# shayneobrien/generative-models

Hardware: AMD Instinct MI355X
Metric: images/sec (28x28 MNIST) per D+G step, NSGAN bs=256 (higher is better)
Workload: dtype f32; 1 GPU; NSGAN MNIST bs=256 fp32 per GPU (BASELINE.json configs[1]); 784-400-20 MLPs, N=50000 synthetic Bernoulli images, parity-mode RNG protocol, Adam 2e-4, D_steps=1; global_batch=256, parallelism=dp1, ranks_seen=1, gradient_exchange=none (1 rank), timing=one 2064-step timed region, cold_start_inclusive=False

## Files before the change

generative_models_amd/csrc/gm_gemm.hip:

```cpp
#include "gm_common.h"
#include "gm_head.h"
#include "gm_gather.h"
#include "gm_dvae.h"
#include "gm_ldsdma.h"

#include <cstdlib>
#include <type_traits>

typedef float f32x16 __attribute__((ext_vector_type(16)));

#ifdef GM_STAMPS
namespace gm_stamps {
constexpr int WAVES = 16, IDS = 40, HDR = 8, MAXB = 512, SLOT_WORDS = HDR + 2 * MAXB + WAVES * IDS * 2, SLOTS = 64;
static unsigned long long* host_buf = nullptr;
static int host_tile = 0, host_next = 0;
struct Ctx { unsigned long long* slot; int tile; };
__device__ __forceinline__ void rec(const Ctx& c, int tile, int id) {
    if (!c.slot || tile != c.tile || (threadIdx.x & 63)) return;
    __builtin_amdgcn_sched_barrier(0);
    unsigned long long* w = c.slot + HDR + 2 * MAXB + ((threadIdx.x >> 6) * IDS + id) * 2;
    w[0] = clock64(); w[1] = wall_clock64();
    __builtin_amdgcn_sched_barrier(0);
}
__device__ __forceinline__ void edge(const Ctx& c, bool exit_, int tile, int M, int N, int K, int mode) {
// ... 156 lines not shown
        float* cp = is_b ? (p.db + m) : (p.C + (int64_t)m * p.ldc + n);
        if (p.accumulate) v += *cp;
        *cp = v;
        if (p.adam.enabled) {
            const int64_t o = is_b ? (int64_t)m : ((int64_t)m * p.ldc + n);
            float* pp = (is_b ? p.adam.pb : p.adam.pW) + o;
            float* mm = (is_b ? p.adam.mb : p.adam.mW) + o;
            float* vv = (is_b ? p.adam.vb : p.adam.vW) + o;
            const int64_t si = gm_slot_index(p.adam.sched_slot);
            const float step_size = p.adam.sched[2 * si], bc2_sqrt = p.adam.sched[2 * si + 1];
            float P = *pp, M = *mm, V = *vv;
            adam_update(P, v, M, V, step_size, bc2_sqrt, p.adam.omb1, p.adam.b2, p.adam.omb2,
                        p.adam.eps, p.adam.wd, p.adam.clamp);
            *pp = P; *mm = M; *vv = V;
            if (kept) *kept = P;
        }
    }
}

__device__ __forceinline__ float4 ld4(const float* q) { return *reinterpret_cast<const float4*>(q); }
__device__ __forceinline__ void st4(float* q, float4 v) { *reinterpret_cast<float4*>(q) = v; }

template <int MODE>
__device__ __forceinline__ void store4(const GemmP& p, float4 v, int m, int n) {
    if (MODE == MODE_FWD) {
        if (p.bias) { const float4 b = ld4(p.bias + n); v.x += b.x; v.y += b.y; v.z += b.z; v.w += b.w; }
        if (p.epi == GM_ACT_RELU) { v.x = fmaxf(v.x, 0.f); v.y = fmaxf(v.y, 0.f); v.z = fmaxf(v.z, 0.f); v.w = fmaxf(v.w, 0.f); }
        else if (p.epi == GM_ACT_SIGMOID) { v.x = gm_sigmoid(v.x); v.y = gm_sigmoid(v.y); v.z = gm_sigmoid(v.z); v.w = gm_sigmoid(v.w); }
        st4(p.C + (int64_t)m * p.ldc + n, v);
        if (p.ip_out && m < p.ip_rows) {
            const float ev = (p.ip_eps + gm_slot_offset(p.ip_slot))[m];
            const float4 x = ld4(p.ip_x + (int64_t)m * p.ip_ldx + n);
            st4(p.ip_out + (int64_t)m * p.ip_ldo + n,
                make_float4(gm_interp_unfused(ev, x.x, v.x), gm_interp_unfused(ev, x.y, v.y),
                            gm_interp_unfused(ev, x.z, v.z), gm_interp_unfused(ev, x.w, v.w)));
        }
    } else if (MODE == MODE_DX) {
        if (p.add) {
            const float4 a = ld4(p.add + (int64_t)m * p.ldadd + n);
            v.x += p.add_scale * a.x; v.y += p.add_scale * a.y; v.z += p.add_scale * a.z; v.w += p.add_scale * a.w;
        }
        if (p.epi == GM_ACT_RELU) {
            const float4 y = ld4(p.aux + (int64_t)m * p.ldaux + n);
            v.x = (y.x > 0.f) ? v.x : 0.f; v.y = (y.y > 0.f) ? v.y : 0.f; v.z = (y.z > 0.f) ? v.z : 0.f; v.w = (y.w > 0.f) ? v.w : 0.f;
        } else if (p.epi == GM_ACT_SIGMOID) {
            const float4 y = ld4(p.aux + (int64_t)m * p.ldaux + n);
            v.x = v.x * (y.x * (1.f - y.x)); v.y = v.y * (y.y * (1.f - y.y));
            v.z = v.z * (y.z * (1.f - y.z)); v.w = v.w * (y.w * (1.f - y.w));
        }
        float* cp = p.C + (int64_t)m * p.ldc + n;
        if (p.accumulate) { const float4 c = ld4(cp); v.x = c.x + v.x; v.y = c.y + v.y; v.z = c.z + v.z; v.w = c.w + v.w; }
        st4(cp, v);
    } else {
        const int64_t o = (int64_t)m * p.ldc + n;
        if (p.accumulate) { const float4 c = ld4(p.C + o); v.x += c.x; v.y += c.y; v.z += c.z; v.w += c.w; }
        st4(p.C + o, v);
        if (p.adam.enabled) {
            const int64_t si = gm_slot_index(p.adam.sched_slot);
            const float step_size = p.adam.sched[2 * si], bc2_sqrt = p.adam.sched[2 * si + 1];
            float4 P = ld4(p.adam.pW + o), M = ld4(p.adam.mW + o), V = ld4(p.adam.vW + o);
            adam_update(P.x, v.x, M.x, V.x, step_size, bc2_sqrt, p.adam.omb1, p.adam.b2, p.adam.omb2, p.adam.eps, p.adam.wd, p.adam.clamp);
            adam_update(P.y, v.y, M.y, V.y, step_size, bc2_sqrt, p.adam.omb1, p.adam.b2, p.adam.omb2, p.adam.eps, p.adam.wd, p.adam.clamp);
            adam_update(P.z, v.z, M.z, V.z, step_size, bc2_sqrt, p.adam.omb1, p.adam.b2, p.adam.omb2, p.adam.eps, p.adam.wd, p.adam.clamp);
            adam_update(P.w, v.w, M.w, V.w, step_size, bc2_sqrt, p.adam.omb1, p.adam.b2, p.adam.omb2, p.adam.eps, p.adam.wd, p.adam.clamp);
            st4(p.adam.pW + o, P); st4(p.adam.mW + o, M); st4(p.adam.vW + o, V);
        }
    }
}

template <int MODE>
__device__ __forceinline__ void store_group(const GemmP& p, float4 v, int m, int n, int ncap) {
    const int nreal = (MODE == MODE_DW) ? p.n_real : p.N;
    if (n + 3 < nreal && n + 3 < ncap) { store4<MODE>(p, v, m, n); return; }
    if (n < p.N && n < ncap) store_element<MODE>(p, v.x, m, n);
    if (n + 1 < p.N && n + 1 < ncap) store_element<MODE>(p, v.y, m, n + 1);
    if (n + 2 < p.N && n + 2 < ncap) store_element<MODE>(p, v.z, m, n + 2);
    if (n + 3 < p.N && n + 3 < ncap) store_element<MODE>(p, v.w, m, n + 3);
}

__device__ __forceinline__ int red_idx(int w, int row, int col) {
    return (w * 32 + row) * 32 + (col ^ ((((row >> 2) ^ row) & 1) << 4));
}

constexpr int KEEP_LD = 68;
template <int MODE, int WAVES, int ROWS = 32, bool LBL = false>
__device__ __forceinline__ void reduce_and_store(const GemmP& p, const float* red, int t, int m0,
                                                 int n0, int ncap = 0x7fffffff, int rcap = 32,
                                                 float* kept = nullptr) {
    if (MODE == MODE_FWD && p.hd_part) {
#pragma unroll
        for (int e = 0; e < 1024 / (WAVES * 64); ++e) {
            const int row = (t >> 5) + e * (WAVES * 2), col = t & 31;
            const bool live = !(ROWS < 32 && row >= ROWS) && row < rcap;
            float v = 0.f;
            if (live) {
#pragma unroll
                for (int ww = 0; ww < WAVES; ++ww) v += red[red_idx(ww, row, col)];
            }
            const int m = m0 + row, n = n0 + col;
            const bool ok = live && m < p.M && n < p.N && n < ncap;
            float pv = 0.f;
            if (ok) {
                const float w = p.hd_w2[n];
                const float y = fwd_value(p, v, n);
                p.C[(int64_t)m * p.ldc + n] = y;
                pv = y * w;
                if (m == 0 && p.hd_snap) {
                    p.hd_snap[n] = w;
                    if (n == 0) p.hd_snap[p.N] = p.hd_b2[0];
                }
            }
#pragma unroll
            for (int o = 16; o > 0; o >>= 1) pv += __shfl_xor(pv, o, 64);
            if (col == 0 && live && m < p.M) p.hd_part[(int64_t)m * p.hd_ldp + (n0 >> 5)] = pv;
        }
        return;
    }
    if (MODE == MODE_FWD && p.sq_part) {
#pragma unroll
        for (int e = 0; e < 1024 / (WAVES * 64); ++e) {
            const int row = (t >> 5) + e * (WAVES * 2), col = t & 31;
            const bool live = !(ROWS < 32 && row >= ROWS) && row < rcap;
            float v = 0.f;
            if (live) {
#pragma unroll
                for (int ww = 0; ww < WAVES; ++ww) v += red[red_idx(ww, row, col)];
            }
            const int m = m0 + row, n = n0 + col;
            const bool ok = live && m < p.M && n < p.N && n < ncap;
            float pv = 0.f;
            if (ok) {
                const float r = fwd_value(p, v, n);
                p.C[(int64_t)m * p.ldc + n] = r;
                const float d = p.sq_x[(int64_t)m * p.sq_ldx + n] - r;
                pv = d * d;
                const float go = -(2.f * d);
                p.sq_dA[(int64_t)m * p.sq_lda + n] = (go * (1.f - r)) * r;
            }
#pragma unroll
            for (int o = 16; o > 0; o >>= 1) pv += __shfl_xor(pv, o, 64);
            if (col == 0 && live && m < p.M) p.sq_part[(int64_t)m * p.sq_ldp + (n0 >> 5)] = pv;
        }
        return;
    }
#pragma unroll
    for (int e = 0; e < 1024 / (WAVES * 64); ++e) {
        const int row = (t >> 5) + e * (WAVES * 2), col = t & 31;
        if ((ROWS < 32 && row >= ROWS) || row >= rcap) continue;
        float v = 0.f;
#pragma unroll
        for (int ww = 0; ww < WAVES; ++ww) v += red[red_idx(ww, row, col)];
        const int m = m0 + row, n = n0 + col;
        if (m >= p.M || n >= p.N || n >= ncap) continue;
        store_element<MODE, LBL>(p, v, m, n, kept ? kept + row * KEEP_LD + col : nullptr);
    }
}

__device__ __forceinline__ float4 keep4(bool ok, float4 v) {
    return make_float4(ok ? v.x : 0.f, ok ? v.y : 0.f, ok ? v.z : 0.f, ok ? v.w : 0.f);
}

template <int NMFMA, int NDSR, int NVMEM, int NDSW>
__device__ __forceinline__ void lds_stage_schedule() {
    constexpr int NMEM = NDSR + NVMEM + NDSW;
    int done = 0;
#pragma unroll
    for (int q = 0; q < NMFMA; ++q) {
        __builtin_amdgcn_sched_group_barrier(0x008, 1, 0);
        const int upto = (NMEM * (q + 1) + NMFMA - 1) / NMFMA;
#pragma unroll
        for (int i = 0; i < 8; ++i) {
            if (done < upto) {
                if (done < NDSR) __builtin_amdgcn_sched_group_barrier(0x100, 1, 0);
                else if (done < NDSR + NVMEM) __builtin_amdgcn_sched_group_barrier(0x020, 1, 0);
                else __builtin_amdgcn_sched_group_barrier(0x200, 1, 0);
                ++done;
            }
        }
    }
}

template <int MODE, int BM, int BN, int WTM, int WTN, int WK, int KU>
struct LdsCfg {
    static constexpr int WM = BM / WTM, WN = BN / WTN, NW = WM * WN * WK, NT = 64 * NW, BK = 8 * WK * KU;
    static constexpr int TI = WTM / 32, TJ = WTN / 32;
    static constexpr bool B_KC = (MODE == MODE_FWD);
    static constexpr int LDK = BK + 4, LDXB = BN + 4;
    static constexpr int A_SZ = BM * LDK;
    static constexpr int B_SZ = B_KC ? BN * LDK : BK * LDXB;
    static constexpr int STAGE = A_SZ + B_SZ;
    static constexpr int NBUF = 3;
    static constexpr int RED = WK * BM * BN;
    static constexpr int FLOATS = (NBUF * STAGE > RED) ? NBUF * STAGE : RED;
};

template <int MODE, int BM, int BN, int WTM, int WTN, int WK, int KU, int PD, int NS>
__global__ __launch_bounds__(64 * (BM / WTM) * (BN / WTN) * WK) void gemm_lds_kernel(GemmP p) {
    using C = LdsCfg<MODE, BM, BN, WTM, WTN, WK, KU>;
    constexpr int NT = C::NT, BK = C::BK, LDK = C::LDK, LDXB = C::LDXB, TI = C::TI, TJ = C::TJ;
    static_assert(MODE != MODE_DW, "forward (A, B k-contiguous) and input gradient (B = W[k][n]) only");
    static_assert(PD >= 2, "two stages are stored before the first barrier");
    __shared__ __attribute__((aligned(16))) float lds[C::FLOATS];

    const int t = threadIdx.x, lane = t & 63, w = t >> 6;
    const int r = lane & 31, h = lane >> 5;
    const int wk = w / (C::WM * C::WN), wmn = w % (C::WM * C::WN), wm = wmn / C::WN, wn = wmn % C::WN;
    const int b = blockIdx.x, xcd = b & 7, l = b >> 3;
    const int tile_m = xcd * p.lds_mpx + l / p.tn, tile_n = l % p.tn;
    if (tile_m >= p.lds_tm) return;
    const int m0 = tile_m * BM, n0 = tile_n * BN;
    const float* A = p.A;
    const float* B = p.B;
#ifdef GM_STAMPS
    const gm_stamps::Ctx st_slot = p.stamp; const int st_tile = (int)blockIdx.x;
#endif
    GM_STAMP_EDGE(p, false, st_tile, MODE + 10);
    GM_STAMP(st_slot, st_tile, 0);

    constexpr int KQ = BK / 4;
    constexpr int XQ = BN / 4;
    constexpr int UA = BM * KQ, CA = (UA + NT - 1) / NT;
    constexpr int UB = C::B_KC ? BN * KQ : BK * XQ, CB = (UB + NT - 1) / NT;
    const float* baseA[CA];
    const float* baseB[CB];
#pragma unroll
    for (int i = 0; i < CA; ++i) {
        const int u = min(t + i * NT, UA - 1);
        baseA[i] = A + (int64_t)min(m0 + u / KQ, p.M - 1) * p.lda + 4 * (u % KQ);
    }
#pragma unroll
    for (int i = 0; i < CB; ++i) {
        const int u = min(t + i * NT, UB - 1);
        if (C::B_KC) baseB[i] = B + (int64_t)min(n0 + u / KQ, p.N - 1) * p.ldb + 4 * (u % KQ);
        else baseB[i] = B + min(n0 + 4 * (u % XQ), p.N - 4);
// ... 150 lines not shown
        GM_STAMP(st_slot, st_tile, 37);
        GM_STAMP_EDGE(p, true, st_tile, MODE + 10);
        return;
    }
    for (int e = t; e < BM * BN; e += NT) {
        const int row = e / BN, col = e % BN;
        float v = 0.f;
#pragma unroll
        for (int kk = 0; kk < WK; ++kk) v += lds[(kk * BM + row) * BN + col];
        const int m = m0 + row, n = n0 + col;
        if (m < p.M && n < p.N) store_element<MODE>(p, v, m, n);
    }
}

inline int lds_pick_cfg(int M, int N) {
    const int bm[2] = {64, 32}, bn[2] = {64, 64}, id[2] = {1, 2};
    long best = -1; int pick = 0;
    for (int i = 0; i < 2; ++i) {
        const long tiles = (long)((M + bm[i] - 1) / bm[i]) * ((N + bn[i] - 1) / bn[i]);
        const long cost = ((tiles + 255) / 256) * bm[i] * bn[i];
        if (best < 0 || cost < best) { best = cost; pick = id[i]; }
    }
    return pick;
}

template <int MODE, int BM, int BN, int WTM, int WTN, int WK, int KU, int PD>
int launch_lds_cfg(hipStream_t s, GemmP p) {
    using C = LdsCfg<MODE, BM, BN, WTM, WTN, WK, KU>;
    const int tm = (p.M + BM - 1) / BM, tn = (p.N + BN - 1) / BN;
    p.lds_tm = tm; p.tn = tn; p.lds_mpx = (tm + 7) / 8;
    const dim3 grid(8 * p.lds_mpx * tn), block(C::NT);
    constexpr int NS784 = (784 + C::BK - 1) / C::BK, NS400 = (400 + C::BK - 1) / C::BK;
    const int S = (p.K + C::BK - 1) / C::BK;
    if (S == NS784) hipLaunchKernelGGL((gemm_lds_kernel<MODE, BM, BN, WTM, WTN, WK, KU, PD, NS784>), grid, block, 0, s, p);
    else if (S == NS400) hipLaunchKernelGGL((gemm_lds_kernel<MODE, BM, BN, WTM, WTN, WK, KU, PD, NS400>), grid, block, 0, s, p);
    else hipLaunchKernelGGL((gemm_lds_kernel<MODE, BM, BN, WTM, WTN, WK, KU, PD, 0>), grid, block, 0, s, p);
    GM_LAUNCH_RET();
}

template <int MODE>
int lds_cfg_for(const GemmP& p, bool vec, bool xv) {
    static_assert(MODE != MODE_DW, "forward and input gradient only");
    constexpr int min_m = 1024;
    if (p.M < min_m || p.K < 64 || !vec || (MODE == MODE_DX && !xv) || p.N < 32) return 0;
    return lds_pick_cfg(p.M, p.N);
}

template <int MODE>
int launch_lds(hipStream_t s, const GemmP& p, int cfg) {
    if (cfg == 1) return launch_lds_cfg<MODE, 64, 64, 32, 64, 4, 1, 4>(s, p);
    return launch_lds_cfg<MODE, 32, 64, 32, 32, 4, 1, 4>(s, p);
}

typedef float f32x4 __attribute__((ext_vector_type(4)));

__device__ __forceinline__ int sigma16(int i) { return ((i & 3) << 2) | ((i >> 2) & 3); }

__device__ __forceinline__ float4 raw_xc4_16(const float* __restrict__ P, int64_t ld, int x0, int X,
                                             int c, int K, int lane) {
    const int e = (lane >> 2) & 3, q = lane & 3, g = lane >> 4;
    const int k = min(16 * c + 4 * g + e, K - 1);
    const int x = min(x0 + 4 * q, X - 4);
    return *reinterpret_cast<const float4*>(P + (int64_t)k * ld + x);
}

__device__ __forceinline__ float dpp_xor8(float v) {
    return __int_as_float(__builtin_amdgcn_mov_dpp(__float_as_int(v), 0x128, 0xF, 0xF, true));
}
__device__ __forceinline__ float dpp_xor4(float v) {
    const int t = __builtin_amdgcn_mov_dpp(__float_as_int(v), 0x141, 0xF, 0xF, true);
    return __int_as_float(__builtin_amdgcn_mov_dpp(t, 0x1B, 0xF, 0xF, true));
}
__device__ __forceinline__ float4 lane48_transpose(float4 v, int lane) {
    const bool b3 = lane & 8, b2 = lane & 4;
    const float s0 = dpp_xor8(b3 ? v.x : v.z), s1 = dpp_xor8(b3 ? v.y : v.w);
    if (b3) { v.x = s0; v.y = s1; } else { v.z = s0; v.w = s1; }
    const float t0 = dpp_xor4(b2 ? v.x : v.y), t1 = dpp_xor4(b2 ? v.z : v.w);
    if (b2) { v.x = t0; v.z = t1; } else { v.y = t0; v.w = t1; }
    return v;
}

template <int W> struct __attribute__((aligned(4))) ILV { float v[W]; };

__device__ __forceinline__ void store2_dw(const GemmP& p, float2 v, int m, int n) {
    const int64_t o = (int64_t)m * p.ldc + n;
    float2* cp = reinterpret_cast<float2*>(p.C + o);
    if (p.accumulate) { const float2 c = *cp; v.x += c.x; v.y += c.y; }
    *cp = v;
    if (p.adam.enabled) {
        const int64_t si = gm_slot_index(p.adam.sched_slot);
        const float step_size = p.adam.sched[2 * si], bc2_sqrt = p.adam.sched[2 * si + 1];
        float2* pp = reinterpret_cast<float2*>(p.adam.pW + o);
        float2* mm = reinterpret_cast<float2*>(p.adam.mW + o);
        float2* vv = reinterpret_cast<float2*>(p.adam.vW + o);
        float2 P = *pp, M = *mm, V = *vv;
        adam_update(P.x, v.x, M.x, V.x, step_size, bc2_sqrt, p.adam.omb1, p.adam.b2, p.adam.omb2, p.adam.eps, p.adam.wd, p.adam.clamp);
        adam_update(P.y, v.y, M.y, V.y, step_size, bc2_sqrt, p.adam.omb1, p.adam.b2, p.adam.omb2, p.adam.eps, p.adam.wd, p.adam.clamp);
        *pp = P; *mm = M; *vv = V;
    }
}

template <int MI, int NI, bool ILO, bool XMAP = false>
__device__ __forceinline__ void dw_reduce_onepass(const GemmP& p, float* red, f32x4 (&acc)[MI][NI], int m0, int n0,
                                                  bool sync_first) {
    constexpr int RT = 16 * MI, CT = 16 * NI, IMG = RT * CT, G = IMG / 2;
    constexpr bool SWZ = !ILO && XMAP && (CT % 32 == 0);
    static_assert(G <= 1024, "one pair of columns per thread");
    const int t = threadIdx.x, lane = t & 63, w = t >> 6;
    const int i16 = lane & 15, g4 = lane >> 4;
    if (sync_first) __syncthreads();
    float* img = red + w * IMG;
#pragma unroll
    for (int e = 0; e < MI; ++e)
#pragma unroll
        for (int f = 0; f < NI; ++f)
#pragma unroll
            for (int r = 0; r < 4; ++r) {
                const int row = ILO ? MI * (4 * g4 + r) + e : 16 * e + (XMAP ? sigma16(4 * g4 + r) : 4 * g4 + r);
                const int col = ILO ? NI * i16 + f : 16 * f + (XMAP ? sigma16(i16) : i16);
                img[row * CT + (SWZ ? col ^ ((row & 1) << 4) : col)] = acc[e][f][r];
            }
    __syncthreads();
#ifdef GM_STAMPS
    const int st_tile = (m0 / RT) * (int)gridDim.x + n0 / CT;
#endif
    GM_STAMP(p.stamp, st_tile, 10);
    if (t >= G) return;
    const int row = t / (CT / 2), c2 = t % (CT / 2);
    float2 v = make_float2(0.f, 0.f);
#pragma unroll
    for (int ww = 0; ww < 16; ++ww) {
        const float2 x = *reinterpret_cast<const float2*>(&red[ww * IMG + row * CT + (SWZ ? (2 * c2) ^ ((row & 1) << 4) : 2 * c2)]);
        v.x += x.x; v.y += x.y;
    }
    GM_STAMP_AFTER(v.x);
    GM_STAMP(p.stamp, st_tile, 11);
    const int m = m0 + row, n = n0 + 2 * c2;
    if (m >= p.M) return;
    if (n + 1 < p.n_real) { store2_dw(p, v, m, n); return; }
    if (n < p.N) store_element<MODE_DW>(p, v.x, m, n);
    if (n + 1 < p.N) store_element<MODE_DW>(p, v.y, m, n + 1);
}

template <int MI, int NI>
__device__ __forceinline__ void dw_il_reduce(const GemmP& p, float* red, f32x4 (&acc)[MI][NI], int m0, int n0,
                                             bool sync_first) {
    constexpr int WAVES = 16;
    if (p.vec_epi) {
        dw_reduce_onepass<MI, NI, true>(p, red, acc, m0, n0, sync_first);
        return;
    }
    const int t = threadIdx.x;
    const int lane = t & 63, w = t >> 6;
    const int i16 = lane & 15, g4 = lane >> 4;
    if (sync_first) __syncthreads();
#pragma unroll
    for (int bm = 0; bm < (MI + 1) / 2; ++bm)
#pragma unroll
        for (int bnk = 0; bnk < (NI + 1) / 2; ++bnk) {
            if (bm + bnk > 0) __syncthreads();
#pragma unroll
            for (int e = 0; e < MI; ++e)
#pragma unroll
                for (int f = 0; f < NI; ++f)
#pragma unroll
                    for (int r = 0; r < 4; ++r) {
                        const int row = MI * (4 * g4 + r) + e, col = NI * i16 + f;
                        if ((row >> 5) == bm && (col >> 5) == bnk)
                            red[red_idx(w, row & 31, col & 31)] = acc[e][f][r];
                    }
            __syncthreads();
            reduce_and_store<MODE_DW, WAVES, (MI > 1 ? 32 : 16)>(p, red, t, m0 + 32 * bm, n0 + 32 * bnk,
                                                                 (2 * bnk + 1 < NI) ? 0x7fffffff : n0 + 32 * bnk + 16,
                                                                 (2 * bm + 1 < MI) ? 32 : 16);
        }
}

template <int MI, int NI, bool OF, int FOLD, bool SL>
__device__ __forceinline__ void gemm16_dw_dma(const GemmP& p, float* red, int bx, int by, float* sds,
                                              const FoldP* fold, int gx) {
    constexpr int WAVES = 16, NP = MI + NI, CH = NP * 256;
    if (gx > 0) {
        const int gy = (p.M + 16 * MI - 1) / (16 * MI), total = gx * gy;
        const int L = by * gx + bx, x = L & 7, k = L >> 3;
        const int base = total >> 3, rem = total & 7;
        const int T = x * base + min(x, rem) + k;
        by = T % gy; bx = T / gy;
    }
    const int t = threadIdx.x, lane = t & 63;
    const int w = __builtin_amdgcn_readfirstlane(t >> 6);
    const int i16 = lane & 15, g4 = lane >> 4;
    const int m0 = by * (16 * MI), n0 = bx * (16 * NI);
#ifdef GM_STAMPS
    const gm_stamps::Ctx st_slot = p.stamp; const int st_tile = by * max(gx, 1) + bx;
#endif
    GM_STAMP_EDGE(p, false, st_tile, MODE_DW + 20);
    GM_STAMP(st_slot, st_tile, 0);
    const int b_cols = p.n_real;
    const int ones_col = p.db ? p.n_real : -1;
    const int nchunks = (p.K + 15) >> 4;
    float* buf = red + w * CH;
    const uint32_t buf_b = (uint32_t)(uintptr_t)buf;
    const int am = m0 + MI * i16, bn = n0 + NI * i16;

    const float* src[NP]; int srow[NP], sld[NP];
#pragma unroll
    for (int j = 0; j < NP; ++j) {
        const bool isA = j < MI;
        const int idx = (isA ? j : j - MI) * 64 + lane;
        const int row = isA ? idx / (4 * MI) : idx / (4 * NI);
        const int c4 = isA ? idx % (4 * MI) : idx % (4 * NI);
        const int col = isA ? min(m0 + 4 * c4, p.M - 4) : min(n0 + 4 * c4, b_cols - 4);
        src[j] = (isA ? slot_base<SL>(p.A, p.a_slot) : slot_base<SL>(p.B, p.b_slot)) + col;
        sld[j] = isA ? (int)p.lda : (int)p.ldb;
        srow[j] = row;
    }
    auto issue = [&](int c) {
#pragma unroll
        for (int j = 0; j < NP; ++j) {
            const int k = min(16 * c + srow[j], p.K - 1);
            slab::glds16(src[j] + (int64_t)k * sld[j], buf_b + j * 1024u);
        }
    };

    float fw[FOLD == 1 ? MI : 1];
    if constexpr (FOLD == 1) {
#pragma unroll
        for (int e = 0; e < MI; ++e) fw[e] = (am + e < p.M) ? p.fold_w2[min(am + e, p.M - 1)] : 0.f;
    }
    f32x4 acc[MI][NI];
#pragma unroll
    for (int e = 0; e < MI; ++e)
#pragma unroll
        for (int f = 0; f < NI; ++f) acc[e][f] = f32x4{0.f, 0.f, 0.f, 0.f};

    const int nq = (nchunks - w + WAVES - 1) / WAVES;
    const bool special = (ones_col >= n0 && ones_col < n0 + 16 * NI) || (p.K & 15) || OF;
    auto run = [&](auto special_tag) {
        constexpr bool SPECIAL = decltype(special_tag)::value;
        if (nq > 0) issue(w);
        GM_STAMP(st_slot, st_tile, 17);
        if constexpr (FOLD == 1) fold_fill_lds(*fold, sds, fold->R);
        for (int q = 0; q < nq; ++q) {
            const int c = w + q * WAVES;
            slab::wait_vm<0>();
            if (q < 8) GM_STAMP(st_slot, st_tile, 20 + 2 * q);
            ILV<MI> ra[4]; ILV<NI> rb[4];
#pragma unroll
            for (int s = 0; s < 4; ++s) {
                const int row = 4 * s + g4;
                ra[s] = *reinterpret_cast<const ILV<MI>*>(buf + row * (16 * MI) + MI * i16);
                rb[s] = *reinterpret_cast<const ILV<NI>*>(buf + 256 * MI + row * (16 * NI) + NI * i16);
            }
            slab::wait_lgkm0();
            if (q + 1 < nq) issue(c + WAVES);
#pragma unroll
            for (int s = 0; s < 4; ++s) {
                const int k = 16 * c + 4 * s + g4;
                float fa[MI], fb[NI];
#pragma unroll
                for (int e = 0; e < MI; ++e) {
                    float v = ra[s].v[e];
                    if constexpr (FOLD == 1) v = (v > 0.f) ? sds[min(k, p.K - 1)] * fw[e] : 0.f;
                    if constexpr (SPECIAL) v = (k < p.K) ? v : 0.f;
                    fa[e] = v;
                }
#pragma unroll
                for (int f = 0; f < NI; ++f) {
                    float v = rb[s].v[f];
                    if constexpr (SPECIAL) {
                        float one = 1.f;
                        if constexpr (OF) one = (k >= p.ones_from) ? 1.f : 0.f;
                        v = (bn + f == ones_col) ? one : v;
                    }
                    fb[f] = v;
                }
#pragma unroll
                for (int e = 0; e < MI; ++e)
#pragma unroll
                    for (int f = 0; f < NI; ++f)
                        acc[e][f] = __builtin_amdgcn_mfma_f32_16x16x4f32(fa[e], fb[f], acc[e][f], 0, 0, 0);
            }
            GM_STAMP_AFTER(acc[MI - 1][NI - 1][0]);
            if (q < 8) GM_STAMP(st_slot, st_tile, 21 + 2 * q);
        }
    };
    if (special) run(std::true_type{}); else run(std::false_type{});
    GM_STAMP(st_slot, st_tile, 9);
    dw_il_reduce<MI, NI>(p, red, acc, m0, n0, true);
    GM_STAMP(st_slot, st_tile, 12);
    GM_STAMP_EDGE(p, true, st_tile, MODE_DW + 20);
}

template <int MODE, bool DMA, int MI, int NI> struct RedSize {
    static constexpr int base = 16 * 32 * 32;
    static constexpr int onepass = (MODE == MODE_DW && MI * NI > 4) ? 16 * 256 * MI * NI : 0;
    static constexpr int dma = (MODE == MODE_DW && DMA) ? 16 * (MI + NI) * 256 : 0;
    static constexpr int m1 = base > onepass ? base : onepass;
    static constexpr int value = m1 > dma ? m1 : dma;
};

template <int MODE, bool VEC, int WAVES, int G, bool XV, int MI, int NI, bool OF = false, int FOLD = 0, bool DMA = false,
          bool TP = false, bool PK = false, bool SL = true, bool LBL = false>
__device__ __forceinline__ void gemm16_body(const GemmP& p, float* red, int bx, int by,
                                            float* sds = nullptr, const FoldP* fold = nullptr, int gx = 0,
                                            float* kept = nullptr) {
    static_assert(!TP || (FOLD == 1 && !DMA), "two-phase losses: folded weight gradient, operands through registers");
    static_assert(FOLD == 0 || (FOLD == 1 && MODE == MODE_DW && XV) || (FOLD == 2 && MODE == MODE_DX && VEC),
                  "folded head: 16-byte operand paths only");
    static_assert(G == 1, "per-chunk schedule (G stays in the kernel names so that they keep their shape across rounds)");
    static_assert(!PK || (WAVES == 16 && !DMA && ((MODE == MODE_FWD && VEC) || (MODE == MODE_DW && XV))),
                  "bit-packed operand rows: 16-byte operand paths through registers only");
    if constexpr (DMA && MODE == MODE_DW && XV && WAVES == 16 && FOLD != 2) {
        gemm16_dw_dma<MI, NI, OF, FOLD, SL>(p, red, bx, by, sds, fold, gx);
        return;
    }
    const int t = threadIdx.x;
    const int lane = t & 63, w = t >> 6;
    const int i16 = lane & 15, g4 = lane >> 4;
    const int m0 = by * (16 * MI), n0 = bx * (16 * NI);
#ifdef GM_STAMPS
    const gm_stamps::Ctx st_slot = p.stamp; const int st_tile = by * (int)gridDim.x + bx;
#endif
    GM_STAMP_EDGE(p, false, st_tile, MODE);
    GM_STAMP(st_slot, st_tile, 0);

    const float* A = slot_base<SL>(p.A, p.a_slot);
    const float* B = slot_base<SL>(p.B, p.b_slot);
    const int b_cols = (MODE == MODE_DW) ? p.n_real : p.N;
    const int ones_col = (MODE == MODE_DW && p.db) ? p.n_real : -1;
    const int nchunks = (p.K + 15) >> 4;
    GM_STAMP_AFTER(A); GM_STAMP_AFTER(B); GM_STAMP_AFTER(nchunks);
    GM_STAMP(st_slot, st_tile, 16);

    float4 fw[FOLD == 1 ? MI : 1];
    float fds[FOLD == 2 ? MI : 1];
    const int xq_ld = lane & 3, xe_ld = (lane >> 2) & 3;
    constexpr bool XMAP_A = MODE == MODE_DW && XV, XMAP_B = MODE != MODE_FWD && XV;
    const int ia = XMAP_A ? sigma16(i16) : i16, ib = XMAP_B ? sigma16(i16) : i16;
    if constexpr (FOLD == 1) {
#pragma unroll
        for (int mi = 0; mi < MI; ++mi)
            fw[mi] = *reinterpret_cast<const float4*>(
                p.fold_w2 + min(m0 + 16 * mi + 4 * xq_ld, p.M - 4));
    }
    auto load_a = [&](int c, int mi) -> float4 {
        const int kb = 16 * c + 4 * g4, x0 = m0 + 16 * mi;
        if (MODE == MODE_DW) {
            if (XV) return raw_xc4_16(A, p.lda, x0, p.M, c, p.K, lane);
            return raw_xc(A, p.lda, x0 + i16, p.M, kb, p.K);
        }
        return raw_kc<VEC>(A, p.lda, x0 + i16, p.M, kb, p.K);
    };
    auto load_b = [&](int c, int ni) -> float4 {
        const int kb = 16 * c + 4 * g4, x0 = n0 + 16 * ni;
        if (MODE == MODE_FWD) return raw_kc<VEC>(B, p.ldb, x0 + i16, p.N, kb, p.K);
        if (XV) return raw_xc4_16(B, p.ldb, x0, b_cols, c, p.K, lane);
        return raw_xc(B, p.ldb, x0 + i16, b_cols, kb, p.K);
    };
    auto fix_a = [&](float4 v, int c, int mi, float4 wk) -> float4 {
        const int kb = 16 * c + 4 * g4, x = m0 + 16 * mi + ia;
        if constexpr (FOLD == 1)
            v = fold_dh4(v, sds[min(16 * c + 4 * g4 + xe_ld, p.K - 1)], fw[mi]);
        if constexpr (FOLD == 2) v = fold_dh4(v, fds[mi], wk);
        if (MODE == MODE_DW)
            return fix_xc(XV ? lane48_transpose(v, lane) : v, x, p.M, kb, p.K, -1);
        return fix_kc(v, x, p.M, kb, p.K);
    };
    auto fix_b = [&](float4 v, int c, int ni) -> float4 {
        const int kb = 16 * c + 4 * g4, x = n0 + 16 * ni + ib;
        if (MODE == MODE_FWD) return fix_kc(v, x, p.N, kb, p.K);
        return fix_xc(XV ? lane48_transpose(v, lane) : v, x, b_cols, kb, p.K, ones_col, OF ? p.ones_from : 0);
    };

    f32x4 acc[MI][NI];
#pragma unroll
    for (int mi = 0; mi < MI; ++mi)
#pragma unroll
        for (int ni = 0; ni < NI; ++ni) acc[mi][ni] = f32x4{0.f, 0.f, 0.f, 0.f};

    const int nq = (nchunks - w + WAVES - 1) / WAVES;
    auto consume = [&](const float4 (&ra)[MI], const float4 (&rb)[NI], float4 wk, int q) {
        const int cq = w + q * WAVES;
        float4 fa[MI], fb[NI];
#pragma unroll
        for (int mi = 0; mi < MI; ++mi) fa[mi] = fix_a(ra[mi], cq, mi, wk);
#pragma unroll
        for (int ni = 0; ni < NI; ++ni) fb[ni] = fix_b(rb[ni], cq, ni);
        GM_STAMP_AFTER(fa[MI - 1].x); GM_STAMP_AFTER(fb[NI - 1].x);
        if (q < 4) GM_STAMP(st_slot, st_tile, 1 + 2 * q);
#pragma unroll
        for (int mi = 0; mi < MI; ++mi)
#pragma unroll
            for (int ni = 0; ni < NI; ++ni) {
                f32x4 c4 = acc[mi][ni];
                c4 = __builtin_amdgcn_mfma_f32_16x16x4f32(fa[mi].x, fb[ni].x, c4, 0, 0, 0);
                c4 = __builtin_amdgcn_mfma_f32_16x16x4f32(fa[mi].y, fb[ni].y, c4, 0, 0, 0);
                c4 = __builtin_amdgcn_mfma_f32_16x16x4f32(fa[mi].z, fb[ni].z, c4, 0, 0, 0);
                c4 = __builtin_amdgcn_mfma_f32_16x16x4f32(fa[mi].w, fb[ni].w, c4, 0, 0, 0);
                acc[mi][ni] = c4;
            }
        GM_STAMP_AFTER(acc[MI - 1][NI - 1][0]);
        if (q < 4) GM_STAMP(st_slot, st_tile, 2 + 2 * q);
    };
    auto load_wk = [&](int cc) -> float4 {
        if constexpr (FOLD == 2) return *reinterpret_cast<const float4*>(p.fold_w2 + min(16 * cc + 4 * g4, p.K - 4));
        return make_float4(0.f, 0.f, 0.f, 0.f);
    };
    auto fold_prologue = [&]() {
        if constexpr (FOLD == 1) {
            if constexpr (TP) {
                FoldTP tp_unused;
                fold_fill_lds_tp(*fold, sds, fold->R, tp_unused);
            } else {
#ifdef GM_STAMPS
                {
                    for (int r = threadIdx.x; r < fold->R; r += blockDim.x) {
                        float s_ = fold_score(*fold, r);
                        GM_STAMP_AFTER(s_);
                        if (r == (int)threadIdx.x) GM_STAMP(st_slot, st_tile, 14);
                        float ds_, l_;
                        fold_row(*fold, r, s_, ds_, l_);
                        sds[r] = ds_;
                    }
                    GM_STAMP(st_slot, st_tile, 15);
                    __syncthreads();
                }
#else
                fold_fill_lds(*fold, sds, fold->R);
#endif
            }
        } else if constexpr (FOLD == 2) {
            if (t < 16 * MI) {
                float s_, ds_, l_;
                fold_row(*fold, min(m0 + t, fold->R - 1), s_, ds_, l_);
                sds[t] = ds_;
            }
            GM_STAMP(st_slot, st_tile, 15);
            __syncthreads();
#pragma unroll
            for (int mi = 0; mi < MI; ++mi) fds[mi] = sds[16 * mi + i16];
        }
    };
    if constexpr (PK) {
        constexpr int PN = MODE == MODE_FWD ? MI : NI;
        auto pk_elem = [&](int c, int j) -> int {
            return MODE == MODE_FWD ? min(16 * c + 4 * g4, p.K - 4) : min(n0 + 16 * j + 4 * xq_ld, b_cols - 4);
        };
        auto load_pk = [&](int c, int j) -> uint32_t {
            const int row = MODE == MODE_FWD ? m0 + 16 * j + i16 : 16 * c + 4 * g4 + xe_ld;
            return p.pk_bits[(int64_t)row * p.pk_wpr + (pk_elem(c, j) >> 5)];
        };
        const int nq_s = __builtin_amdgcn_readfirstlane(nq);
        int q_pk;
        if (MODE == MODE_FWD) q_pk = (m0 < p.pk_rows) ? nq_s : 0;
        else q_pk = min(nq_s, max(0, ((p.pk_rows >> 4) - __builtin_amdgcn_readfirstlane(w) + WAVES - 1) / WAVES));
        auto do_chunk = [&](auto is_pk, auto with_prologue, int q) {
            constexpr bool P = decltype(is_pk)::value;
            float4 ra[MI], rb[NI];
            uint32_t pw[PN];
            const int cc = w + q * WAVES;
#pragma unroll
            for (int mi = 0; mi < MI; ++mi) {
                if constexpr (P && MODE == MODE_FWD) pw[mi] = load_pk(cc, mi);
                else ra[mi] = load_a(cc, mi);
            }
#pragma unroll
            for (int ni = 0; ni < NI; ++ni) {
                if constexpr (P && MODE == MODE_DW) pw[ni] = load_pk(cc, ni);
                else rb[ni] = load_b(cc, ni);
            }
            const float4 wk = load_wk(cc);
            if constexpr (decltype(with_prologue)::value) fold_prologue();
            if constexpr (P) {
#pragma unroll
                for (int j = 0; j < PN; ++j) {
                    const float4 x = pk_expand(pw[j], pk_elem(cc, j));
                    if constexpr (MODE == MODE_FWD) ra[j] = x; else rb[j] = x;
                }
            }
            consume(ra, rb, wk, q);
        };
        constexpr std::true_type yes{};
        constexpr std::false_type no{};
        int q0 = 0;
        if constexpr (FOLD != 0) {
            if (nq_s > 0) { if (q_pk > 0) do_chunk(yes, yes, 0); else do_chunk(no, yes, 0); }
            else fold_prologue();
            q0 = 1;
        }
        for (int q = q0; q < q_pk; ++q) do_chunk(yes, no, q);
        for (int q = max(q0, q_pk); q < nq_s; ++q) do_chunk(no, no, q);
    } else {
    int q_first = 0;
    if constexpr (FOLD != 0) {
        float4 ra[MI], rb[NI];
        float4 wk = make_float4(0.f, 0.f, 0.f, 0.f);
        const bool have = nq > 0;
        float4 pv[4];
        if constexpr (FOLD == 1 && !TP) {
            if (t < fold->R) fold_part_load(*fold, t, pv);
        }
        if constexpr (FOLD == 2) {
            if (t < 16 * MI) fold_part_load(*fold, min(m0 + t, fold->R - 1), pv);
        }
        if (have) {
#pragma unroll
            for (int mi = 0; mi < MI; ++mi) ra[mi] = load_a(w, mi);
#pragma unroll
            for (int ni = 0; ni < NI; ++ni) rb[ni] = load_b(w, ni);
            wk = load_wk(w);
        }
        GM_STAMP(st_slot, st_tile, 17);
        if constexpr (FOLD == 1 && !TP) fold_fill_lds_pre(*fold, sds, fold->R, pv);
        else if constexpr (FOLD == 2) {
            if (t < 16 * MI) {
                float s_, ds_, l_;
                fold_row_of(*fold, min(m0 + t, fold->R - 1), fold_score_of(*fold, pv), s_, ds_, l_);
                sds[t] = ds_;
            }
            GM_STAMP(st_slot, st_tile, 15);
            __syncthreads();
#pragma unroll
            for (int mi = 0; mi < MI; ++mi) fds[mi] = sds[16 * mi + i16];
        }
        else fold_prologue();
        GM_STAMP(st_slot, st_tile, 13);
        if (have) consume(ra, rb, wk, 0);
        q_first = 1;
    }
    for (int q = q_first; q < nq; ++q) {
        float4 ra[MI], rb[NI];
        const int cc = w + q * WAVES;
#pragma unroll
        for (int mi = 0; mi < MI; ++mi) ra[mi] = load_a(cc, mi);
#pragma unroll
        for (int ni = 0; ni < NI; ++ni) rb[ni] = load_b(cc, ni);
        const float4 wk = load_wk(cc);
        consume(ra, rb, wk, q);
    }
    }
    GM_STAMP(st_slot, st_tile, 9);
    if constexpr (MODE == MODE_DW && WAVES == 16 && MI * NI > 4) {
        if (p.vec_epi) {
            dw_reduce_onepass<MI, NI, false, XMAP_A>(p, red, acc, m0, n0, false);
            GM_STAMP(st_slot, st_tile, 12);
            GM_STAMP_EDGE(p, true, st_tile, MODE);
            return;
        }
    }
#pragma unroll
    for (int bm = 0; bm < (MI + 1) / 2; ++bm)
#pragma unroll
        for (int bn = 0; bn < (NI + 1) / 2; ++bn) {
            if (bm + bn > 0) __syncthreads();
#pragma unroll
            for (int rgi = 0; rgi < 4; ++rgi) {
                const int row = XMAP_A ? sigma16(g4 * 4 + rgi) : g4 * 4 + rgi;
                red[red_idx(w, row, ib)] = acc[2 * bm][2 * bn][rgi];
                if (2 * bn + 1 < NI) red[red_idx(w, row, 16 + ib)] = acc[2 * bm][(2 * bn + 1 < NI) ? 2 * bn + 1 : 0][rgi];
                if (2 * bm + 1 < MI) {
                    constexpr int MIX = MI > 1 ? MI - 1 : 0;
                    const int mu = (2 * bm + 1 < MI) ? 2 * bm + 1 : MIX;
                    red[red_idx(w, 16 + row, ib)] = acc[mu][2 * bn][rgi];
                    if (2 * bn + 1 < NI)
                        red[red_idx(w, 16 + row, 16 + ib)] = acc[mu][(2 * bn + 1 < NI) ? 2 * bn + 1 : 0][rgi];
                }
            }
            __syncthreads();
            if (bm + bn == 0) GM_STAMP(st_slot, st_tile, 10);
            reduce_and_store<MODE, WAVES, (MI > 1 ? 32 : 16), LBL>(p, red, t, m0 + 32 * bm, n0 + 32 * bn,
                                                              (2 * bn + 1 < NI) ? 0x7fffffff : n0 + 32 * bn + 16,
                                                              (2 * bm + 1 < MI) ? 32 : 16,
                                                              kept ? kept + 32 * bm * KEEP_LD + 32 * bn : nullptr);
        }
    GM_STAMP(st_slot, st_tile, 12);
    GM_STAMP_EDGE(p, true, st_tile, MODE);
}

template <int MODE, bool VEC, int WAVES, int G, bool XV, int MI, int NI, bool DMA = false, bool SL = false>
__global__ __launch_bounds__(WAVES * 64) void gemm16_kernel(GemmP p) {
    __shared__ __attribute__((aligned(16))) float red[(WAVES == 16) ? RedSize<MODE, DMA, MI, NI>::value : WAVES * 32 * 32];
    gemm16_body<MODE, VEC, WAVES, G, XV, MI, NI, false, 0, DMA, false, false, SL>(p, red, blockIdx.x, blockIdx.y, nullptr, nullptr,
                                                                                  (int)gridDim.x);
}

template <bool VEC, int MI, int NI>
__global__ __launch_bounds__(1024) void gemm16_fwd_label_kernel(GemmP p) {
    __shared__ __attribute__((aligned(16))) float red[RedSize<MODE_FWD, false, MI, NI>::value];
    gemm16_body<MODE_FWD, VEC, 16, 1, false, MI, NI, false, 0, false, false, false, false, true>(p, red, blockIdx.x, blockIdx.y,
                                                                                                nullptr, nullptr, (int)gridDim.x);
}

template <int MODE, bool VEC, int G, bool XV, int MI, int NI, bool OF = false, bool FOLDED = false, bool DMA = false,
          bool TP = false, bool PK = false>
__device__ __forceinline__ void gemm16_with_head(const GemmP& p, const HeadBwdP& hp, int hrows,
                                                 int hblocks) {
    __shared__ __attribute__((aligned(16))) float red[RedSize<MODE, DMA, MI, NI>::value];
    __shared__ float sds[FOLDED ? FOLD_MAX_ROWS : 1];
    constexpr int FOLD = FOLDED ? (MODE == MODE_DW ? 1 : 2) : 0;
    if ((int)blockIdx.y < hrows) {
        const int bid = blockIdx.y * gridDim.x + blockIdx.x;
        if (bid < hblocks) head_bwd_body<TP>(hp, bid, sds);
        return;
    }
    gemm16_body<MODE, VEC, 16, G, XV, MI, NI, OF, FOLD, DMA, TP, PK, false>(p, red, blockIdx.x, blockIdx.y - hrows, sds, &hp.fold,
                                                                            (int)gridDim.x);
}

template <bool VEC, int G, bool XV, int MI, int NI, bool OF = false, bool FOLDED = false, bool DMA = false>
__global__ __launch_bounds__(1024) void gemm16_dw_head_kernel(GemmP p, HeadBwdP hp, int hrows,
                                                              int hblocks) {
    gemm16_with_head<MODE_DW, VEC, G, XV, MI, NI, OF, FOLDED, DMA>(p, hp, hrows, hblocks);
}

__global__ __launch_bounds__(1024) void gemm16_fwd_bits_kernel(GemmP p) {
    __shared__ __attribute__((aligned(16))) float red[RedSize<MODE_FWD, false, 2, 2>::value];
    gemm16_body<MODE_FWD, true, 16, 1, false, 2, 2, false, 0, false, false, true, false>(p, red, blockIdx.x, blockIdx.y);
}
__global__ __launch_bounds__(1024) void gemm16_dw_head_bits_kernel(GemmP p, HeadBwdP hp, int hrows, int hblocks) {
    gemm16_with_head<MODE_DW, false, 1, true, 2, 3, false, true, false, false, true>(p, hp, hrows, hblocks);
}

template <int MI, int NI>
__global__ __launch_bounds__(1024) void gemm16_dw_head_tp_kernel(GemmP p, HeadBwdP hp, int hrows, int hblocks) {
// ... 872 lines not shown
```

Before: 4.207 million images/sec.

## Load contiguous per-lane strips for DW/DX GEMM operands and remap the reduction

```diff
diff --git a/generative_models_amd/csrc/gm_gemm.hip b/generative_models_amd/csrc/gm_gemm.hip
--- a/generative_models_amd/csrc/gm_gemm.hip
+++ b/generative_models_amd/csrc/gm_gemm.hip
@@ -262,11 +262,15 @@
     return (w * 32 + row) * 32 + (col ^ ((((row >> 2) ^ row) & 1) << 4));
 }
 
+__device__ __forceinline__ int red_idx_sx(int w, int row, int col, int flip) {
+    return (w * 32 + row) * 32 + (col ^ flip);
+}
+
 constexpr int KEEP_LD = 68;
-template <int MODE, int WAVES, int ROWS = 32, bool LBL = false>
+template <int MODE, int WAVES, int ROWS = 32, bool LBL = false, int SXD = 0>
 __device__ __forceinline__ void reduce_and_store(const GemmP& p, const float* red, int t, int m0,
                                                  int n0, int ncap = 0x7fffffff, int rcap = 32,
-                                                 float* kept = nullptr) {
+                                                 float* kept = nullptr, int srow0 = 0) {
     if (MODE == MODE_FWD && p.hd_part) {
 #pragma unroll
         for (int e = 0; e < 1024 / (WAVES * 64); ++e) {
@@ -329,7 +333,8 @@
         if ((ROWS < 32 && row >= ROWS) || row >= rcap) continue;
         float v = 0.f;
 #pragma unroll
-        for (int ww = 0; ww < WAVES; ++ww) v += red[red_idx(ww, row, col)];
+        for (int ww = 0; ww < WAVES; ++ww)
+            v += red[SXD > 0 ? red_idx_sx(ww, row, col, ((srow0 + row) / (SXD > 0 ? SXD : 1)) & 1) : red_idx(ww, row, col)];
         const int m = m0 + row, n = n0 + col;
         if (m >= p.M || n >= p.N || n >= ncap) continue;
         store_element<MODE, LBL>(p, v, m, n, kept ? kept + row * KEEP_LD + col : nullptr);
@@ -646,6 +651,31 @@
 
 template <int W> struct __attribute__((aligned(4))) ILV { float v[W]; };
 
+template <int W> struct __attribute__((aligned(W == 4 ? 16 : W == 2 ? 8 : 4))) XSV { float v[W]; };
+
+template <int W>
+__device__ __forceinline__ XSV<W> raw_xs(const float* __restrict__ P, int64_t ld, int xl, int X, int k, int K) {
+    return *reinterpret_cast<const XSV<W>*>(P + (int64_t)min(k, K - 1) * ld + min(xl, X - W));
+}
+template <int W, bool FOLD>
+__device__ __forceinline__ void fix_xs(const XSV<W>& r, float (&o)[W], int xl, int X, bool kin, int ones_col, float one,
+                                       float ds, const float* fw) {
+    float c[W];
+#pragma unroll
+    for (int s = 0; s < W; ++s) c[s] = r.v[s];
+    if constexpr (W == 3) {
+        const int d = xl - min(xl, X - 3);
+        c[0] = (d == 0) ? r.v[0] : ((d == 1) ? r.v[1] : r.v[2]);
+        c[1] = (d == 0) ? r.v[1] : r.v[2];
+    }
+#pragma unroll
+    for (int s = 0; s < W; ++s) {
+        float v = c[s];
+        if constexpr (FOLD) v = (v > 0.f) ? ds * fw[s] : 0.f;
+        o[s] = kin ? ((xl + s < X) ? v : ((xl + s == ones_col) ? one : 0.f)) : 0.f;
+    }
+}
+
 __device__ __forceinline__ void store2_dw(const GemmP& p, float2 v, int m, int n) {
     const int64_t o = (int64_t)m * p.ldc + n;
     float2* cp = reinterpret_cast<float2*>(p.C + o);
@@ -664,11 +694,13 @@
     }
 }
 
-template <int MI, int NI, bool ILO, bool XMAP = false>
+template <int MI, int NI, bool ILO, bool XMAP = false, bool SX = false>
 __device__ __forceinline__ void dw_reduce_onepass(const GemmP& p, float* red, f32x4 (&acc)[MI][NI], int m0, int n0,
                                                   bool sync_first) {
     constexpr int RT = 16 * MI, CT = 16 * NI, IMG = RT * CT, G = IMG / 2;
-    constexpr bool SWZ = !ILO && XMAP && (CT % 32 == 0);
+    constexpr bool SWZ = !ILO && !SX && XMAP && (CT % 32 == 0);
+    constexpr bool SXZ = SX && (NI % 2 == 0);
+    static_assert(!SX || !ILO, "one accumulator layout");
     static_assert(G <= 1024, "one pair of columns per thread");
     const int t = threadIdx.x, lane = t & 63, w = t >> 6;
     const int i16 = lane & 15, g4 = lane >> 4;
@@ -680,9 +712,11 @@
         for (int f = 0; f < NI; ++f)
 #pragma unroll
             for (int r = 0; r < 4; ++r) {
-                const int row = ILO ? MI * (4 * g4 + r) + e : 16 * e + (XMAP ? sigma16(4 * g4 + r) : 4 * g4 + r);
-                const int col = ILO ? NI * i16 + f : 16 * f + (XMAP ? sigma16(i16) : i16);
-                img[row * CT + (SWZ ? col ^ ((row & 1) << 4) : col)] = acc[e][f][r];
+                const int row = SX ? 16 * e + 4 * r + g4
+                                   : ILO ? MI * (4 * g4 + r) + e : 16 * e + (XMAP ? sigma16(4 * g4 + r) : 4 * g4 + r);
+                const int col = (SX || ILO) ? NI * i16 + f : 16 * f + (XMAP ? sigma16(i16) : i16);
+                const int cs = SXZ ? col ^ (((col >> 5) & 1) << 1) ^ (row & 1) : SWZ ? col ^ ((row & 1) << 4) : col;
+                img[row * CT + cs] = acc[e][f][r];
             }
     __syncthreads();
 #ifdef GM_STAMPS
@@ -690,15 +724,18 @@
 #endif
     GM_STAMP(p.stamp, st_tile, 10);
     if (t >= G) return;
-    const int row = t / (CT / 2), c2 = t % (CT / 2);
+    const int lrow = t / (CT / 2), c2 = t % (CT / 2);
+    const int cr = SXZ ? (2 * c2) ^ (((c2 >> 4) & 1) << 1) : SWZ ? (2 * c2) ^ ((lrow & 1) << 4) : 2 * c2;
     float2 v = make_float2(0.f, 0.f);
 #pragma unroll
     for (int ww = 0; ww < 16; ++ww) {
-        const float2 x = *reinterpret_cast<const float2*>(&red[ww * IMG + row * CT + (SWZ ? (2 * c2) ^ ((row & 1) << 4) : 2 * c2)]);
+        const float2 x = *reinterpret_cast<const float2*>(&red[ww * IMG + lrow * CT + cr]);
         v.x += x.x; v.y += x.y;
     }
+    if (SXZ && (lrow & 1)) v = make_float2(v.y, v.x);
     GM_STAMP_AFTER(v.x);
     GM_STAMP(p.stamp, st_tile, 11);
+    const int row = SX ? MI * sigma16(lrow & 15) + (lrow >> 4) : lrow;
     const int m = m0 + row, n = n0 + 2 * c2;
     if (m >= p.M) return;
     if (n + 1 < p.n_real) { store2_dw(p, v, m, n); return; }
@@ -856,6 +893,43 @@
     GM_STAMP_EDGE(p, true, st_tile, MODE_DW + 20);
 }
 
+template <int MODE, int MI, int NI>
+constexpr bool sx_feed() {
+    return (MODE == MODE_DW && !(MI == 1 && NI > 2)) || MODE == MODE_DX;
+}
+
+template <int MODE, int MI, int NI, bool ILA>
+__device__ __forceinline__ void sx_block_reduce(const GemmP& p, float* red, f32x4 (&acc)[MI][NI], int m0, int n0,
+                                                float* kept) {
+    const int t = threadIdx.x;
+    const int lane = t & 63, w = t >> 6;
+    const int i16 = lane & 15, g4 = lane >> 4;
+    constexpr int SXD = ILA ? 4 * MI : 4;
+#pragma unroll
+    for (int bm = 0; bm < (MI + 1) / 2; ++bm)
+#pragma unroll
+        for (int bn = 0; bn < (NI + 1) / 2; ++bn) {
+            if (bm + bn > 0) __syncthreads();
+#pragma unroll
+            for (int e = 0; e < MI; ++e)
+#pragma unroll
+                for (int f = 0; f < NI; ++f)
+#pragma unroll
+                    for (int r = 0; r < 4; ++r) {
+                        const int row = ILA ? MI * (4 * g4 + r) + e : 16 * e + 4 * g4 + r, col = NI * i16 + f;
+                        const bool rin = ILA ? (MI <= 2 || (row >> 5) == bm) : (e >> 1) == bm;
+                        if (rin && (NI <= 2 || (col >> 5) == bn))
+                            red[red_idx_sx(w, row & 31, col & 31, g4 & 1)] = acc[e][f][r];
+                    }
+            __syncthreads();
+            reduce_and_store<MODE, 16, (MI > 1 ? 32 : 16), false, SXD>(p, red, t, m0 + 32 * bm, n0 + 32 * bn,
+                                                                       (2 * bn + 1 < NI) ? 0x7fffffff : n0 + 32 * bn + 16,
+                                                                       (2 * bm + 1 < MI) ? 32 : 16,
+                                                                       kept ? kept + 32 * bm * KEEP_LD + 32 * bn : nullptr,
+                                                                       ILA ? 32 * bm : 0);
+        }
+}
+
 template <int MODE, bool DMA, int MI, int NI> struct RedSize {
     static constexpr int base = 16 * 32 * 32;
     static constexpr int onepass = (MODE == MODE_DW && MI * NI > 4) ? 16 * 256 * MI * NI : 0;
@@ -897,30 +971,47 @@
     GM_STAMP_AFTER(A); GM_STAMP_AFTER(B); GM_STAMP_AFTER(nchunks);
     GM_STAMP(st_slot, st_tile, 16);
 
+    constexpr bool SX = XV && WAVES == 16 && !PK && (MODE == MODE_DW || MODE == MODE_DX) && sx_feed<MODE, MI, NI>();
+    constexpr bool SXA = SX && MODE == MODE_DW;
+    using FragA = std::conditional_t<SXA, XSV<MI>, float4>;
+    using FragB = std::conditional_t<SX, XSV<NI>, float4>;
+    constexpr int NA = SXA ? 4 : MI, NB = SX ? 4 : NI;
+    const int xla = m0 + MI * i16, xlb = n0 + NI * i16;
+
     float4 fw[FOLD == 1 ? MI : 1];
+    float fws[FOLD == 1 ? MI : 1];
     float fds[FOLD == 2 ? MI : 1];
     const int xq_ld = lane & 3, xe_ld = (lane >> 2) & 3;
     constexpr bool XMAP_A = MODE == MODE_DW && XV, XMAP_B = MODE != MODE_FWD && XV;
     const int ia = XMAP_A ? sigma16(i16) : i16, ib = XMAP_B ? sigma16(i16) : i16;
-    if constexpr (FOLD == 1) {
+    if constexpr (FOLD == 1 && SX) {
+#pragma unroll
+        for (int mi = 0; mi < MI; ++mi) fws[mi] = p.fold_w2[min(xla + mi, p.M - 1)];
+    } else if constexpr (FOLD == 1) {
 #pragma unroll
         for (int mi = 0; mi < MI; ++mi)
             fw[mi] = *reinterpret_cast<const float4*>(
                 p.fold_w2 + min(m0 + 16 * mi + 4 * xq_ld, p.M - 4));
     }
-    auto load_a = [&](int c, int mi) -> float4 {
+    auto load_a = [&](int c, int mi) -> FragA {
         const int kb = 16 * c + 4 * g4, x0 = m0 + 16 * mi;
-        if (MODE == MODE_DW) {
-            if (XV) return raw_xc4_16(A, p.lda, x0, p.M, c, p.K, lane);
-            return raw_xc(A, p.lda, x0 + i16, p.M, kb, p.K);
-        }
-        return raw_kc<VEC>(A, p.lda, x0 + i16, p.M, kb, p.K);
+        if constexpr (SXA) return raw_xs<MI>(A, p.lda, xla, p.M, kb + mi, p.K);
+        else {
+            if (MODE == MODE_DW) {
+                if (XV) return raw_xc4_16(A, p.lda, x0, p.M, c, p.K, lane);
+                return raw_xc(A, p.lda, x0 + i16, p.M, kb, p.K);
+            }
+            return raw_kc<VEC>(A, p.lda, x0 + i16, p.M, kb, p.K);
+        }
     };
-    auto load_b = [&](int c, int ni) -> float4 {
+    auto load_b = [&](int c, int ni) -> FragB {
         const int kb = 16 * c + 4 * g4, x0 = n0 + 16 * ni;
-        if (MODE == MODE_FWD) return raw_kc<VEC>(B, p.ldb, x0 + i16, p.N, kb, p.K);
-        if (XV) return raw_xc4_16(B, p.ldb, x0, b_cols, c, p.K, lane);
-        return raw_xc(B, p.ldb, x0 + i16, b_cols, kb, p.K);
+        if constexpr (SX) return raw_xs<NI>(B, p.ldb, xlb, b_cols, kb + ni, p.K);
+        else {
+            if (MODE == MODE_FWD) return raw_kc<VEC>(B, p.ldb, x0 + i16, p.N, kb, p.K);
+            if (XV) return raw_xc4_16(B, p.ldb, x0, b_cols, c, p.K, lane);
+            return raw_xc(B, p.ldb, x0 + i16, b_cols, kb, p.K);
+        }
     };
     auto fix_a = [&](float4 v, int c, int mi, float4 wk) -> float4 {
         const int kb = 16 * c + 4 * g4, x = m0 + 16 * mi + ia;
@@ -944,8 +1035,43 @@
         for (int ni = 0; ni < NI; ++ni) acc[mi][ni] = f32x4{0.f, 0.f, 0.f, 0.f};
 
     const int nq = (nchunks - w + WAVES - 1) / WAVES;
-    auto consume = [&](const float4 (&ra)[MI], const float4 (&rb)[NI], float4 wk, int q) {
+    auto consume = [&](const FragA (&ra)[NA], const FragB (&rb)[NB], float4 wk, int q) {
         const int cq = w + q * WAVES;
+        if constexpr (SX) {
+            float fa[4][MI], fb[4][NI];
+            if constexpr (!SXA) {
+#pragma unroll
+                for (int mi = 0; mi < MI; ++mi) {
+                    const float4 v = fix_a(ra[mi], cq, mi, wk);
+                    fa[0][mi] = v.x; fa[1][mi] = v.y; fa[2][mi] = v.z; fa[3][mi] = v.w;
+                }
+            }
+#pragma unroll
+            for (int t4 = 0; t4 < 4; ++t4) {
+                const int k = 16 * cq + 4 * g4 + t4;
+                const bool kin = k < p.K;
+                if constexpr (SXA) {
+                    float ds = 0.f;
+                    if constexpr (FOLD == 1) ds = sds[min(k, p.K - 1)];
+                    fix_xs<MI, FOLD == 1>(ra[t4], fa[t4], xla, p.M, kin, -1, 0.f, ds, fws);
+                }
+                float one = 1.f;
+                if constexpr (OF) one = (k >= p.ones_from) ? 1.f : 0.f;
+                fix_xs<NI, false>(rb[t4], fb[t4], xlb, b_cols, kin, ones_col, one, 0.f, nullptr);
+            }
+            GM_STAMP_AFTER(fa[3][MI - 1]); GM_STAMP_AFTER(fb[3][NI - 1]);
+            if (q < 4) GM_STAMP(st_slot, st_tile, 1 + 2 * q);
+#pragma unroll
+            for (int mi = 0; mi < MI; ++mi)
+#pragma unroll
+                for (int ni = 0; ni < NI; ++ni) {
+                    f32x4 c4 = acc[mi][ni];
+#pragma unroll
+                    for (int t4 = 0; t4 < 4; ++t4)
+                        c4 = __builtin_amdgcn_mfma_f32_16x16x4f32(fa[t4][mi], fb[t4][ni], c4, 0, 0, 0);
+                    acc[mi][ni] = c4;
+                }
+        } else {
         float4 fa[MI], fb[NI];
 #pragma unroll
         for (int mi = 0; mi < MI; ++mi) fa[mi] = fix_a(ra[mi], cq, mi, wk);
@@ -964,6 +1090,7 @@
                 c4 = __builtin_amdgcn_mfma_f32_16x16x4f32(fa[mi].w, fb[ni].w, c4, 0, 0, 0);
                 acc[mi][ni] = c4;
             }
+        }
         GM_STAMP_AFTER(acc[MI - 1][NI - 1][0]);
         if (q < 4) GM_STAMP(st_slot, st_tile, 2 + 2 * q);
     };
@@ -1058,7 +1185,7 @@
     } else {
     int q_first = 0;
     if constexpr (FOLD != 0) {
-        float4 ra[MI], rb[NI];
+        FragA ra[NA]; FragB rb[NB];
         float4 wk = make_float4(0.f, 0.f, 0.f, 0.f);
         const bool have = nq > 0;
         float4 pv[4];
@@ -1070,9 +1197,9 @@
         }
         if (have) {
 #pragma unroll
-            for (int mi = 0; mi < MI; ++mi) ra[mi] = load_a(w, mi);
-#pragma unroll
-            for (int ni = 0; ni < NI; ++ni) rb[ni] = load_b(w, ni);
+            for (int mi = 0; mi < NA; ++mi) ra[mi] = load_a(w, mi);
+#pragma unroll
+            for (int ni = 0; ni < NB; ++ni) rb[ni] = load_b(w, ni);
             wk = load_wk(w);
         }
         GM_STAMP(st_slot, st_tile, 17);
@@ -1094,17 +1221,31 @@
         q_first = 1;
     }
     for (int q = q_first; q < nq; ++q) {
-        float4 ra[MI], rb[NI];
+        FragA ra[NA]; FragB rb[NB];
         const int cc = w + q * WAVES;
 #pragma unroll
-        for (int mi = 0; mi < MI; ++mi) ra[mi] = load_a(cc, mi);
-#pragma unroll
-        for (int ni = 0; ni < NI; ++ni) rb[ni] = load_b(cc, ni);
+        for (int mi = 0; mi < NA; ++mi) ra[mi] = load_a(cc, mi);
+#pragma unroll
+        for (int ni = 0; ni < NB; ++ni) rb[ni] = load_b(cc, ni);
         const float4 wk = load_wk(cc);
         consume(ra, rb, wk, q);
     }
     }
     GM_STAMP(st_slot, st_tile, 9);
+    if constexpr (SX) {
+        if constexpr (MODE == MODE_DW && MI * NI > 4) {
+            if (p.vec_epi) {
+                dw_reduce_onepass<MI, NI, false, false, true>(p, red, acc, m0, n0, false);
+                GM_STAMP(st_slot, st_tile, 12);
+                GM_STAMP_EDGE(p, true, st_tile, MODE);
+                return;
+            }
+        }
+        sx_block_reduce<MODE, MI, NI, SXA>(p, red, acc, m0, n0, kept);
+        GM_STAMP(st_slot, st_tile, 12);
+        GM_STAMP_EDGE(p, true, st_tile, MODE);
+        return;
+    }
     if constexpr (MODE == MODE_DW && WAVES == 16 && MI * NI > 4) {
         if (p.vec_epi) {
             dw_reduce_onepass<MI, NI, false, XMAP_A>(p, red, acc, m0, n0, false);
```

Result: faster. 4.333 million images/sec (median of 6 runs) (+3.0%).
